# xultaeculcis/climate-super-resolution

Measured on NVIDIA B200. Metric: generator_inference_hr_mpixel_per_s, higher is better.
Workload: dtype bf16

## Files before the change

climate-super-resolution_b200/csrc/api.cu:

```cuda
#include <algorithm>
#include <atomic>
#include <cstdarg>
#include <cstdio>
#include <cstring>
#include <map>
#include <mutex>
#include <string>
#include <vector>

#include "../../include/climsr_b200.h"
#include "conv_tc.cuh"
#include "disc.cuh"
#include "elementwise.cuh"
#include "loss.cuh"
#include "metrics.cuh"
#include "rcan.cuh"
#include "rdb_tc.cuh"
#include "wgrad_tc.cuh"

namespace csr {

static thread_local char g_err[512] = "";
static std::atomic<long long> g_launches{0};
static int g_opt_pdl = 1;
static long long* g_trace = nullptr;
static unsigned long long* g_timeline = nullptr;
static int g_timeline_cap = 0;
static int g_opt_force_sw = 0;
static int g_opt_max_slots = 8;
static int g_opt_no_tma_store = 0;
static int g_opt_two_acc = 0;
static int g_opt_force_generic = 0;
static int g_opt_one_mma = 0;
static int g_opt_graphs = 1;
static int g_opt_graph_max_px = 1 << 21;
static int g_opt_issue_order = 1;
static int g_opt_wgrad_atomic = 1;
static int g_opt_eight_acc = 1;
static int g_opt_tall = 1;
static int g_opt_narrow_box = 1;
static int g_opt_regroup = 0;
static int g_opt_trace_cta = 0;
static int g_opt_reserve_sms = 0;
static int g_opt_l2_prefetch = 0;
static int g_dbg_dense = 0;
static int g_opt_dense_min = 2;
static int g_opt_tap_pack = 1;
static int g_opt_hyb = 1;
static int g_opt_merge_phases = 1;
static int g_opt_fuse_tail = 3;
[[maybe_unused]] static int g_opt_dense9 = 0;
static int g_opt_dense = 1;
static int g_opt_early = 1;
static int g_opt_pair = 0;
static int g_opt_no_single_group = 3;
static int g_dbg_wgrad[5] = {0, 0, 0, 0, 0};
static int g_opt_no_direct32 = 1;

static int fail(int code, const char* fmt, ...) {
  va_list ap;
  va_start(ap, fmt);
  vsnprintf(g_err, sizeof(g_err), fmt, ap);
  va_end(ap);
  return code;
}
#define CSR_CUDA(expr)                                                                          \
  do {                                                                                          \
    cudaError_t _e = (expr);                                                                    \
    if (_e != cudaSuccess) return fail(CSR_ERR_CUDA, "%s: %s", #expr, cudaGetErrorString(_e)); \
  } while (0)

static inline size_t align_up(size_t v, size_t a) { return (v + a - 1) / a * a; }
static inline int ceil_div(int a, int b) { return (a + b - 1) / b; }

struct DeviceInfo {
  bool ok = false;
  int sms = 0;
  int dev = -1;
};
static int device_info(DeviceInfo* out) {
  int dev = 0;
  CSR_CUDA(cudaGetDevice(&dev));
  static DeviceInfo cache[64];
  static std::mutex mu;
  if (dev >= 0 && dev < 64) {
    std::lock_guard<std::mutex> lock(mu);
    if (cache[dev].ok) { *out = cache[dev]; return CSR_OK; }
  }
  int major = 0, minor = 0, sms = 0;
  CSR_CUDA(cudaDeviceGetAttribute(&major, cudaDevAttrComputeCapabilityMajor, dev));
  CSR_CUDA(cudaDeviceGetAttribute(&minor, cudaDevAttrComputeCapabilityMinor, dev));
  CSR_CUDA(cudaDeviceGetAttribute(&sms, cudaDevAttrMultiProcessorCount, dev));
  if (major != 10) return fail(CSR_ERR_UNSUPPORTED, "device %d is sm_%d%d; this library is sm_100a only", dev, major, minor);
  out->ok = true;
  out->sms = sms;
  out->dev = dev;
  if (dev >= 0 && dev < 64) {
    std::lock_guard<std::mutex> lock(mu);
    cache[dev] = *out;
  }
  return CSR_OK;
}

typedef CUresult (*EncodeTiledFn)(CUtensorMap*, CUtensorMapDataType, cuuint32_t, void*, const cuuint64_t*, const cuuint64_t*,
                                  const cuuint32_t*, const cuuint32_t*, CUtensorMapInterleave, CUtensorMapSwizzle,
                                  CUtensorMapL2promotion, CUtensorMapFloatOOBfill);
// ... 281 lines not shown
    }
  }
  if (!p.pair && tma_out && tl.n_slots < 2 * p.n_kblocks && pp.n_store % 16 == 0 && io.out_C % 16 == 0 && (io.out_coff + pp.co_lo) % 16 == 0 &&
      !g_opt_no_direct32) {
    Tiling t2;
    if (choose_tiling(H, W, pp.kh, pp.kw, p.w_bytes, p.n_kblocks, 0, 0, &t2, p.box_c * 2) == CSR_OK && t2.n_slots >= 2 * p.n_kblocks) {
      tl = t2;
      p.store_mode = kStoreDirect32;
      p.stage_row_bytes = 0;
    }
  }
  p.act = io.act;
  if (io.act_upto > 0 && io.act == CSR_ACT_LRELU02) {
    const int upto = io.act_upto - pp.co_lo;
    if (upto <= 0) p.act = CSR_ACT_NONE;
    else if (upto < pp.n_store) { p.act = 3; p.act_upto = upto; }
  }
  p.n_stage = p.n_groups;
  const bool early_plain = res_bits == 0 && p.n_groups == 1 &&
      ((p.KW == 3 && p.PW == 1 && (p.act == 0 || p.act == 1 || p.act == 3)) || (p.KW == 2 && p.PW <= 1 && p.act == 1) ||
       (p.KW == 1 && p.PW == 0 && p.act == 2));
  const bool early_res = g_opt_early >= 2 && (res_bits == 1 || res_bits == 3) && !io.r1_pre && p.KW == 3 && p.PW == 1 && p.act == 0 && p.n_groups <= 2;
  if (g_opt_early && !p.pair && !p.tall_shift && tma_out && p.npad == 64 && pp.n_store == 64 && !g_opt_force_generic && (early_plain || early_res)) {
    Tiling te2, te1;
    const bool ok2 = choose_tiling(H, W, pp.kh, pp.kw, p.w_bytes, p.n_kblocks, p.stage_row_bytes, 2, &te2, p.box_c * 2) == CSR_OK;
    const bool ok1 = choose_tiling(H, W, pp.kh, pp.kw, p.w_bytes, p.n_kblocks, p.stage_row_bytes, 1, &te1, p.box_c * 2) == CSR_OK;
    const int want = std::min(2 * p.n_kblocks, 4);
    int stages = 0;
    if (ok2 && te2.n_slots >= want) stages = 2;
    else if (ok1 && (!ok2 || te1.n_slots > te2.n_slots)) stages = 1;
    else if (ok2) stages = 2;
    const Tiling& te = stages == 1 ? te1 : te2;
    if (stages && te.n_slots >= std::min(2, p.n_kblocks + 1) && (early_plain || te.n_slots > tl.n_slots || te.n_slots >= want)) {
      tl = te;
      p.early = 1;
      p.n_groups = 1;
      p.n_stage = stages;
      if (4 * p.KW * p.npad <= 512 && !g_opt_two_acc) p.n_acc = 4;
    }
  }
  {
    const bool hyb_early = (g_opt_hyb & 1) && p.early && ((p.KW == 3 && p.PW == 1) || (p.KW == 2 && p.PW <= 1));
#ifdef CSR_EXPERIMENTS
    const bool hyb_res = (g_opt_hyb & 2) && !p.early && p.KW == 3 && p.PW == 1 && p.act == 0 && (res_bits == 1 || res_bits == 3) && !io.r1_pre &&
                         p.n_groups == 2;
#else
    const bool hyb_res = false;
#endif
    if ((hyb_early || hyb_res) && !p.pair && !p.tall_shift && p.store_mode == kStoreStaged && p.npad == 64 && pp.n_store == 64 && p.box_c == 64 &&
        !p.stream_w && !g_opt_force_generic) {
      p.hyb = 1;
      const int acc_cols = (p.KW - 1) * p.npad;
      if (4 * acc_cols <= 512 && !g_opt_two_acc && (p.early || (g_opt_hyb & 4))) p.n_acc = 4;
    }
  }
  p.SW = tl.SW; p.TH = tl.TH; p.TW = tl.TW;
  p.sw_shift = 0;
  while ((1 << p.sw_shift) < p.SW) ++p.sw_shift;
  p.tiles_x = ceil_div(W, p.TW);
  p.tiles_y = ceil_div(H, p.TH << p.tall_shift);
  p.num_tiles = p.tiles_x * p.tiles_y * N;
  p.tiles_per_img = p.tiles_x * p.tiles_y;
  if ((long long)p.tiles_x * p.tiles_y * N >= (1 << 24) || p.tiles_per_img >= (1 << 16))
    return fail(CSR_ERR_UNSUPPORTED, "too many tiles (%d x %d x %d) for one launch", p.tiles_x, p.tiles_y, N);
  p.magic_img = ((1ull << 40) / (unsigned)p.tiles_per_img) + 1;
  p.magic_row = ((1ull << 40) / (unsigned)p.tiles_x) + 1;
  p.win_rows = tl.win_rows; p.win_bytes = tl.win_bytes; p.slot_bytes = tl.slot_bytes; p.n_slots = tl.n_slots;
  p.win_slot_bytes = (int)align_up(tl.win_bytes, 1024);
  p.stage_bytes = tl.stage_bytes;
  p.n_mma = g_opt_one_mma ? 1 : 2;
  p.issue_order = (p.n_mma == 2) && (g_opt_issue_order == 2 || (g_opt_issue_order == 1 && p.pair));
  int cols = 32;
  while (cols < p.n_acc * (p.hyb ? p.KW - 1 : p.KW) * p.npad) cols *= 2;
  if (cols > 512 || p.KW * p.npad > 256) return fail(CSR_ERR_UNSUPPORTED, "KW*npad = %d exceeds the UMMA N / TMEM budget", p.KW * p.npad);
  p.tmem_cols = cols;
  p.trace = g_trace;
  p.trace_cta = g_opt_trace_cta;
  p.use_pdl = g_opt_pdl;
  p.l2_prefetch = ((size_t)N * H * W * io.in_C * 2 > (size_t)48 << 20) ? g_opt_l2_prefetch : 0;
  p.force_generic = g_opt_force_generic;
  p.r1_pre = io.r1 ? io.r1_pre : 0;
  p.s1 = io.s1; p.s2 = io.s2;
  p.r1 = io.r1; p.r1_C = io.r1_C; p.r1_coff = io.r1_coff + pp.co_lo;
  p.r2 = io.r2; p.r2_C = io.r2_C; p.r2_coff = io.r2_coff + pp.co_lo;
  p.gate = io.gate; p.gate_C = io.gate_C; p.gate_coff = io.gate_coff + pp.co_lo; p.gate_from = io.gate_from - pp.co_lo; p.gate_neg = io.gate_neg;
  if ((io.r1 || io.r2 || io.gate) && up != 1) return fail(CSR_ERR_UNSUPPORTED, "residual / gate operands are not supported on nearest-x2 layers");
  p.out = io.out; p.out_C = io.out_C; p.out_coff = io.out_coff + pp.co_lo;
  p.out_sy = p.out_sx = up;
  p.out_oy = pp.phase >= 0 ? (pp.phase >> 1) : 0;
  p.out_ox = pp.phase >= 0 ? (pp.phase & 1) : 0;
  p.out_H = up * H; p.out_W = up * W;
  cl->w_off = pp.w_off; cl->b_off = pp.b_off;
  if (conv_smem_bytes(p) > (size_t)kSmemLimit) return fail(CSR_ERR_UNSUPPORTED, "conv needs %zu bytes of shared memory", conv_smem_bytes(p));
  return encode_act_map(&cl->tmap, io.in, N, H, W, io.in_C, p.SW, p.win_rows, p.box_c);
}

struct WgradLaunch {
  WgradParams p;
  CUtensorMap tx0, tx1, tg0, tg1;
};

static int build_wgrad(int sms, int N, int H, int W, int KW, int PW, int dy_off, int n_dy, const void* x, int x_C, int xc0, const void* gA, int gA_C,
                       int gA_c0, const void* gB, int gB_C, int gB_c0, int n_cols, float* dacc, long part_stride, int ld_n, WgradLaunch* wl) {
  if (n_cols % 16 || n_cols < 16 || n_cols > 128) return fail(CSR_ERR_UNSUPPORTED, "wgrad: n_cols %d", n_cols);
  if (x_C % 8 || gA_C % 8 || xc0 % 8 || gA_c0 % 8) return fail(CSR_ERR_BAD_ARG, "wgrad: channel pitch/offset must be multiples of 8");
  WgradParams& p = wl->p;
// ... 437 lines not shown
          ConvLaunch stub;
          memset(&stub.p, 0, sizeof(stub.p));
          stub.dense = (int)P->dense.size();
          P->dense.push_back(dl);
          P->convs.push_back(stub);
          li += 4;
          goto conv5;
        }
      }
      for (int k = 1; k <= 4; ++k) {
        ConvIO io = io_of(src, C, src, C, nf + (k - 1) * gc, CSR_ACT_LRELU02);
        if (g_opt_regroup) {
          if (k == 1) {
            io.act_upto = gc;
          } else {
            io.cin_off = nf;
            io.r1 = src; io.r1_C = C; io.r1_coff = nf + (k - 1) * gc; io.r1_pre = 1;
          }
        }
        rc = add(h, w, io);
        if (rc) return rc;
      }
    conv5:
      ConvIO io = io_of(src, C, dst, C, 0, CSR_ACT_NONE);
      io.r1 = src; io.r1_C = C; io.s1 = 0.2f;
      if (r == 2) { io.r2 = cat(3 * i); io.r2_C = C; io.s2 = 0.2f; }
      rc = add(h, w, io);
      if (rc) return rc;
    }
  }
  void* trunk_out = P->train ? cat(3 * d.nb) : cat(0);
  {
    ConvIO io = io_of(trunk_out, C, t0, 64, 0, CSR_ACT_NONE);
    io.r1 = fea0; io.r1_C = 64; io.s1 = 1.f;
    rc = add(h, w, io);
    if (rc) return rc;
  }
  rc = add(h, w, io_of(t0, 64, m1, 64, 0, CSR_ACT_LRELU02));
  if (rc) return rc;
  rc = add(2 * h, 2 * w, io_of(m1, 64, hrA, 64, 0, CSR_ACT_LRELU02));
  if (rc) return rc;
  const int H = 4 * h, W = 4 * w;
  rc = add(H, W, io_of(hrA, 64, hrB, 64, 0, CSR_ACT_LRELU02));
  if (rc) return rc;
  {
    ConvLaunch& hc = P->convs.back();
    const PackLayer& pt = packs.back();
    bool fused = false;
    if ((g_opt_fuse_tail & 2) && !P->train && hc.p.early && hc.p.KW == 3 && hc.p.PW == 1 && hc.p.npad == 64 && hc.p.stage_row_bytes == 128 &&
        pt.parts.size() == 1 && pt.parts[0].npad == 16 && pt.parts[0].w_bytes == 2048 && pt.cin_pad == 64) {
      ConvParams q = hc.p;
      q.fuse2 = 2; q.w2_bytes = pt.parts[0].w_bytes; q.n2 = 9; q.out2 = hrB; q.out2_plane = (long long)N * H * W;
      if (q.hyb) q.n_acc = 2;
      int cols = 32;
      while (cols < q.n_acc * (q.hyb ? 2 : q.KW) * q.npad + 16) cols *= 2;
      q.tmem_cols = cols;
      if (cols <= 512 && conv_smem_bytes(q) <= (size_t)kSmemLimit && (size_t)9 * N * H * W * sizeof(float) <= (size_t)N * H * W * 64 * 2) {
        hc.p = q;
        hc.w2_off = pt.parts[0].w_off;
        ConvLaunch ts;
        memset(&ts.p, 0, sizeof(ts.p));
        ts.tapsum = 1; ts.taps = reinterpret_cast<const float*>(hrB); ts.tap_plane = (long)N * H * W; ts.tap_H = H; ts.tap_W = W;
        ts.b_off = packs[li].parts[0].b_off;
        P->convs.push_back(ts);
        ++li;
        fused = true;
      }
    }
    if (!fused) {
      ConvIO io = io_of(hrB, 64, P->tlast, 1, 0, CSR_ACT_NONE);
      io.out_kind = kOutF32Planar;
      rc = add(H, W, io);
      if (rc) return rc;
    }
  }
  P->idx_srcnn1 = (int)P->convs.size();
  P->srcnn_pitch = P->train ? 64 : 32;
  const int sp = P->srcnn_pitch;
  rc = add(H, W, io_of(hrC, sp, hrD, 64, 0, CSR_ACT_RELU));
  if (rc) return rc;
  {
    ConvLaunch& c1 = P->convs.back();
    const PackLayer& p2 = packs[li];
    bool fused = false;
    if ((g_opt_fuse_tail & 1) && !P->train && c1.p.early && c1.p.KW == 1 && c1.p.PW == 0 && c1.p.npad == 64 && c1.p.stage_row_bytes == 128 &&
        p2.parts.size() == 1 && p2.parts[0].npad == 32 && p2.parts[0].w_bytes == 4096 && p2.cin_pad == 64 && sp % 8 == 0) {
      ConvParams q = c1.p;
      q.fuse2 = 1; q.w2_bytes = p2.parts[0].w_bytes; q.n2 = 32; q.out2 = hrE; q.out2_C = sp; q.out2_coff = 0;
      int cols = 32;
      while (cols < q.n_acc * q.KW * q.npad + 32) cols *= 2;
      q.tmem_cols = cols;
      if (cols <= 512 && conv_smem_bytes(q) <= (size_t)kSmemLimit) {
        c1.p = q;
        c1.w2_off = p2.parts[0].w_off; c1.b2_off = p2.parts[0].b_off;
        ++li;
        fused = true;
      }
    }
    if (!fused) {
      rc = add(H, W, io_of(hrD, 64, hrE, sp, 0, CSR_ACT_RELU));
      if (rc) return rc;
    }
  }
  {
    ConvIO io = io_of(hrE, sp, nullptr, 1, 0, CSR_ACT_NONE);
    io.out_kind = kOutF32Planar;
// ... 321 lines not shown

using namespace csr;

extern "C" {

int csr_abi_version(void) { return CSR_ABI_VERSION; }
const char* csr_last_error(void) { return g_err; }

int csr_device_check(void) {
  int n = 0;
  cudaError_t e = cudaGetDeviceCount(&n);
  if (e != cudaSuccess || n == 0) return fail(CSR_ERR_CUDA, "no CUDA device: %s", cudaGetErrorString(e));
  DeviceInfo di;
  return device_info(&di);
}

int csr_set_option(int32_t key, int32_t value) {
#ifndef CSR_EXPERIMENTS
  if ((key == 13 && value != 0) || (key == 16 && value != 0) || (key == 8 && value == 0) || (key == 32 && value != 0) || (key == 35 && (value & ~1)))
    return fail(CSR_ERR_UNSUPPORTED, "option %d=%d selects an experimental kernel variant: rebuild with CSR_EXPERIMENTS=1 python build.py --force", key, value);
#endif
  switch (key) {
    case 1: g_opt_pdl = value ? 1 : 0; return CSR_OK;
    case 2: g_opt_force_sw = value; return CSR_OK;
    case 3: g_opt_max_slots = value < 1 ? 1 : value; return CSR_OK;
    case 4: g_opt_no_tma_store = value ? 1 : 0; return CSR_OK;
    case 5: g_opt_two_acc = value ? 1 : 0; return CSR_OK;
    case 6: g_opt_force_generic = value ? 1 : 0; return CSR_OK;
    case 7: g_opt_one_mma = value ? 1 : 0; return CSR_OK;
    case 8: g_opt_no_direct32 = value ? 1 : 0; return CSR_OK;
    case 9: g_opt_no_single_group = value; return CSR_OK;
    case 11: g_opt_graphs = value ? 1 : 0; return CSR_OK;
    case 12: g_opt_graph_max_px = value; return CSR_OK;
    case 13: g_opt_pair = value; return CSR_OK;
    case 14: g_opt_issue_order = value; return CSR_OK;
    case 15: g_opt_trace_cta = value; return CSR_OK;
    case 16: g_opt_regroup = value ? 1 : 0; return CSR_OK;
    case 17: g_opt_narrow_box = value ? 1 : 0; return CSR_OK;
    case 18: g_opt_tall = value ? 1 : 0; return CSR_OK;
    case 19: g_opt_eight_acc = value ? 1 : 0; return CSR_OK;
    case 20: case 21: case 22: case 23: case 24: g_dbg_wgrad[key - 20] = value; return CSR_OK;
    case 25: g_opt_wgrad_atomic = value ? 1 : 0; return CSR_OK;
    case 27: g_opt_dense = value ? 1 : 0; return CSR_OK;
    case 36: g_opt_tap_pack = value ? 1 : 0; return CSR_OK;
    case 35: g_opt_hyb = value; return CSR_OK;
    case 34: g_opt_merge_phases = value ? 1 : 0; return CSR_OK;
    case 33: g_opt_fuse_tail = value & 3; return CSR_OK;
    case 32: g_opt_dense9 = value ? 1 : 0; return CSR_OK;
    case 31: if (value < 0 || value > 64) return fail(CSR_ERR_BAD_ARG, "option 31: windows per SM in [0, 64]"); g_opt_dense_min = value; return CSR_OK;
    case 28: g_dbg_dense = value; return CSR_OK;
    case 29: g_opt_l2_prefetch = value; return CSR_OK;
    case 30: g_opt_reserve_sms = value < 0 ? 0 : value; return CSR_OK;
    case 26: g_opt_early = value; return CSR_OK;
    default: return fail(CSR_ERR_BAD_ARG, "unknown option key %d", key);
  }
}

int64_t csr_kernel_launch_count(void) { return g_launches.load(); }

int csr_has_experiments(void) {
#ifdef CSR_EXPERIMENTS
  return 1;
#else
  return 0;
#endif
}

int csr_debug_set_trace(void* device_buffer) {
#ifdef CSR_ENABLE_TRACE
  g_trace = reinterpret_cast<long long*>(device_buffer);
  return CSR_OK;
#else
  if (!device_buffer) return CSR_OK;
  return fail(CSR_ERR_UNSUPPORTED, "this build has no pipeline tracing (rebuild with CSR_BUILD_TRACE=1 python build.py --force)");
#endif
}

int csr_debug_set_timeline(void* device_u64, int32_t capacity_launches) {
  g_timeline = reinterpret_cast<unsigned long long*>(device_u64);
  g_timeline_cap = device_u64 ? capacity_launches : 0;
  return CSR_OK;
}

int csr_num_layers(const CsrNetDesc* net) {
  int rc = check_net(net);
  if (rc) return rc;
  return (int)layer_table(*net).size();
}

int csr_layer_shape(const CsrNetDesc* net, int32_t i, int32_t shape4[4], char* name, size_t name_cap) {
  int rc = check_net(net);
  if (rc) return rc;
  const auto t = layer_table(*net);
  if (i < 0 || i >= (int)t.size() || !shape4) return fail(CSR_ERR_BAD_ARG, "layer index %d out of range", i);
  shape4[0] = t[i].cout; shape4[1] = t[i].cin; shape4[2] = t[i].kh; shape4[3] = t[i].kw;
  if (name && name_cap) snprintf(name, name_cap, "%s", t[i].name.c_str());
  return CSR_OK;
}

size_t csr_packed_weight_bytes(const CsrNetDesc* net) {
  if (check_net(net)) return 0;
  size_t total = 0;
  const auto t = layer_table(*net);
  pack_layout(fwd_exec_table(*net, t), &total);
  return total;
}
// ... 821 lines not shown
```

climate-super-resolution_b200/csrc/conv_tc.cu:

```cuda
#include <cstdio>

#include "conv_tc.cuh"
#include "ptx.cuh"

namespace csr {

namespace {

#ifdef CSR_ENABLE_TRACE
#define CSR_TRACE(role, tile_it, ev)                                                                                  \
  do {                                                                                                                \
    if (p.trace && blockIdx.x == p.trace_cta && (tile_it) < 64) p.trace[((role) * 64 + (tile_it)) * 8 + (ev)] = clock64();      \
  } while (0)
#else
#define CSR_TRACE(role, tile_it, ev) do { } while (0)
#endif

struct Tile {
  int n, y0, x0;
};

__device__ __forceinline__ int fast_div(int t, unsigned long long magic) {
  return static_cast<int>((static_cast<unsigned long long>(static_cast<unsigned>(t)) * magic) >> 40);
}
// ... 35 lines not shown
    const int src = (lane + delta) & 31;
#pragma unroll
    for (int j = 0; j < 8; ++j) s[j] = __uint_as_float(__shfl_sync(0xffffffffu, raw[j], src));
  }
#pragma unroll
  for (int j = 0; j < 8; j += 2) {
    const float2 t = __fadd2_rn(make_float2(acc[j], acc[j + 1]), make_float2(s[j], s[j + 1]));
    acc[j] = t.x;
    acc[j + 1] = t.y;
  }
}

__device__ __forceinline__ void fma_residual8(float (&v)[8], const uint4& r, float scale) {
  const uint32_t w[4] = {r.x, r.y, r.z, r.w};
#pragma unroll
  for (int i = 0; i < 4; ++i) {
    const float2 t = __ffma2_rn(make_float2(v[2 * i], v[2 * i + 1]), make_float2(scale, scale), make_float2(bf16lo(w[i]), bf16hi(w[i])));
    v[2 * i] = t.x;
    v[2 * i + 1] = t.y;
  }
}

__device__ __forceinline__ void gate8(float (&v)[8], const uint4& g, float neg) {
  const uint32_t w[4] = {g.x, g.y, g.z, g.w};
#pragma unroll
  for (int i = 0; i < 4; ++i) {
    v[2 * i] *= (bf16lo(w[i]) > 0.f) ? 1.f : neg;
    v[2 * i + 1] *= (bf16hi(w[i]) > 0.f) ? 1.f : neg;
  }
}

__device__ __forceinline__ uint4 ldg16(const void* base, size_t pix, int C, int coff) {
  return __ldg(reinterpret_cast<const uint4*>(reinterpret_cast<const __nv_bfloat16*>(base) + pix * C + coff));
}

}

template <int KW_T, int PW_T, int ACT_T, int RES_T, int ST_T, int PAIR_T = 0, int TALL_T = 0, int EARLY_T = 0, int FUSE_T = 0, int HYB_T = 0>
__global__ void __launch_bounds__(kConvThreads, 1)
conv_tc_kernel(const ConvParams p, const __grid_constant__ CUtensorMap tmap) {
  extern __shared__ uint8_t smem_raw[];
  const uint32_t smem_base = (smem_u32(smem_raw) + 1023u) & ~1023u;
  const uint32_t slots_addr = smem_base;
  const uint32_t stage_addr = slots_addr + static_cast<uint32_t>(p.n_slots) * p.slot_bytes;
  const uint32_t w_addr = stage_addr + static_cast<uint32_t>(p.n_stage) * p.stage_bytes;
  const uint32_t crank = PAIR_T ? cluster_ctarank() : 0u;
  const int w_local = p.stream_w ? 0 : (PAIR_T ? (p.w_bytes >> 1) : p.w_bytes);
  const uint32_t w2_addr = w_addr + ((w_local + 127) & ~127);
  const uint32_t b2_addr = w2_addr + (FUSE_T ? static_cast<uint32_t>(p.w2_bytes) : 0u);
  const uint32_t bias_addr = b2_addr + (FUSE_T ? 128u : 0u);
  const uint32_t bar_addr = bias_addr + 256;
  const int S = p.n_slots;
  const int NA = p.n_acc;
  const int NG = p.n_groups;
  const int wpg = kEpilogueWarps / NG;
  auto bar_w = bar_addr;
  auto bar_a_full = [&](int s) { return bar_addr + 8u * (1 + s); };
  auto bar_a_empty = [&](int s) { return bar_addr + 8u * (1 + S + s); };
  auto bar_acc_full = [&](int b) { return bar_addr + 8u * (1 + 2 * S + b); };
  auto bar_acc_empty = [&](int b) { return bar_addr + 8u * (9 + 2 * S + b); };
  auto bar_token = [&](int w) { return bar_addr + 8u * (17 + 2 * S + w); };
  const uint32_t bar_d2 = bar_addr + 8u * (19 + 2 * S);
  const uint32_t tmem_slot_addr = bar_addr + 8u * (20 + 2 * S);
  const uint32_t lead_off = PAIR_T ? (map_to_cta(bar_addr, 0) - bar_addr) : 0u;
  uint8_t* smem_gen = smem_raw + (smem_base - smem_u32(smem_raw));
  float* bias_s = reinterpret_cast<float*>(smem_gen + (bias_addr - smem_base));
  volatile uint32_t* tmem_slot = reinterpret_cast<volatile uint32_t*>(smem_gen + (tmem_slot_addr - smem_base));
  volatile uint32_t* progress = tmem_slot + 1;

  const int warp = threadIdx.x >> 5;
  const int lane = threadIdx.x & 31;
  const int KW = KW_T ? KW_T : p.KW;
  const int ph_eff = p.PH + static_cast<int>(blockIdx.y) * p.part_ph;
  const int oy_eff = p.out_oy + static_cast<int>(blockIdx.y) * p.part_oy;

  griddep_launch_dependents();

  if (threadIdx.x == 0) {
    progress[0] = 0;
    progress[1] = 0;
    mbar_init(bar_token(0), 1);
    mbar_init(bar_token(1), 1);
    mbar_init(bar_d2, 1);
    tma_prefetch_desc(&tmap);
    mbar_init(bar_w, (PAIR_T && crank == 0) ? 2 : 1);
    for (int s = 0; s < S; ++s) {
      mbar_init(bar_a_full(s), 1);
      mbar_init(bar_a_empty(s), 1);
    }
    for (int b = 0; b < NA; ++b) {
      mbar_init(bar_acc_full(b), 1);
      mbar_init(bar_acc_empty(b), PAIR_T ? 2 * wpg : wpg);
    }
    fence_mbar_init();
    fence_proxy_async_smem();
  }
  if constexpr (PAIR_T) cluster_sync_all();
  if (threadIdx.x == 0 && !p.stream_w) {
    const uint8_t* wsrc = reinterpret_cast<const uint8_t*>(p.wpk) + static_cast<size_t>(blockIdx.y) * p.part_w_bytes;
    if constexpr (PAIR_T) {
      const int full = (KW_T ? KW_T : p.KW) * p.npad * 32, half = full >> 1;
      mbar_arrive_expect_tx(bar_w, w_local);
      for (int off = 0, loc = 0; off < p.w_bytes; off += full, loc += half)
        bulk_load(w_addr + loc, wsrc + off + crank * half, half, bar_w);
    } else {
      mbar_arrive_expect_tx(bar_w, p.w_bytes + (FUSE_T ? p.w2_bytes : 0));
      for (int off = 0; off < p.w_bytes; off += 32768) {
// ... 161 lines not shown
              }
              if (last_kb && hh == 0) umma_commit(bar_acc_full(buf));
            }
          }
          if (last_kb) CSR_TRACE(1, it, 4);
          if constexpr (PAIR_T) {
            umma_commit_pair(bar_a_empty(slot));
            if (last_kb) umma_commit_pair(bar_acc_full(buf));
          } else {
            umma_commit(bar_a_empty(slot));
            if (last_kb) umma_commit(bar_acc_full(buf + tall - 1));
          }
          if (kb == p.n_kblocks - 1) CSR_TRACE(1, it, 5);
        }
        __syncwarp();
        if (kb == p.n_kblocks - 1 && lane == 0) {
          if (p.issue_order) mbar_arrive(bar_token(mw));
          CSR_TRACE(1, it, 3);
        }
        ring_advance(1);
      }
      if (p.n_mma > 1) {
        ring_advance(p.n_kblocks);
        entry += p.n_kblocks;
      }
      buf += p.n_mma * tall;
      if (buf >= NA) { buf -= NA; acc_phase ^= 1; }
      if (lane == 0) CSR_TRACE(1, it, 6);
    }
  } else {
    const int ew = warp - 1 - kMmaWarps;
    const int g = ew / wpg;
    const int wj = ew - g * wpg;
    const int lane_grp = warp & 3;
    const int sub = wj >> 2;
    const int cstep = wpg >> 2;
    const int gthreads = wpg * 32;
    const bool tracer = (ew == 0 && lane == 0);
    const int m = lane_grp * 32 + lane;
    const int ty = m >> p.sw_shift;
    const int tx = m & (p.SW - 1);
    const int n_chunks = ST_T == 3 ? 1 : p.npad >> 3;
    const int PW = KW_T ? PW_T : p.PW;
    const bool col_ok = (tx >= PW) && (tx < PW + p.TW);
    const int srow = ty * p.TW + (tx - PW);
    const int act = ACT_T >= 0 ? ACT_T : p.act;
    const bool has_r1 = RES_T >= 0 ? (RES_T & 1) != 0 : p.r1 != nullptr;
    const bool has_r2 = RES_T >= 0 ? (RES_T & 2) != 0 : p.r2 != nullptr;
    const bool has_gate = RES_T >= 0 ? (RES_T & 4) != 0 : p.gate != nullptr;
    const bool r1_pre = RES_T >= 0 ? (RES_T & 8) != 0 : p.r1_pre != 0;
    const bool tma_store = ST_T >= 0 ? ST_T == 1 : (p.store_mode == kStoreStaged);
    const bool need_pix = !tma_store || has_r1 || has_r2 || has_gate;
    const uint32_t swz = (p.stage_row_bytes == 128) ? static_cast<uint32_t>(srow & 7) : 0u;
    const uint32_t srow_addr = stage_addr + static_cast<uint32_t>(g) * p.stage_bytes + static_cast<uint32_t>(srow * p.stage_row_bytes);
    const uint32_t sbuf = stage_addr + static_cast<uint32_t>(g) * p.stage_bytes;
    const uint32_t t_lane = tmem_base + (static_cast<uint32_t>(lane_grp * 32) << 16);
    const int d0 = -PW, d1 = 1 - PW, d2 = 2 - PW;
    const int rp = p.stage_row_bytes >> 4;
    const int n_pieces = p.TH * p.TW * rp;
    uint32_t pc_s[4], pc_d[4], pc_yx[4];
    if (tma_store) {
      const int tid_g = wj * 32 + lane;
#pragma unroll
      for (int k = 0; k < 4; ++k) {
        const int i = tid_g + k * gthreads;
        const int sr = i / rp, c = i - sr * rp;
        const int dy = sr / p.TW, dx = sr - dy * p.TW;
        const uint32_t z = (p.stage_row_bytes == 128) ? static_cast<uint32_t>(sr & 7) : 0u;
        pc_s[k] = sbuf + static_cast<uint32_t>(sr * p.stage_row_bytes) + ((static_cast<uint32_t>(c) ^ z) << 4);
        pc_d[k] = static_cast<uint32_t>((dy * p.out_sy * p.out_W + dx * p.out_sx) * p.out_C + c * 8);
        pc_yx[k] = (i < n_pieces) ? ((static_cast<uint32_t>(dy) << 16) | static_cast<uint32_t>(dx)) : 0xffffffffu;
      }
    }
    int buf = g % NA;
    uint32_t acc_phase = 0;
    if constexpr (EARLY_T) {
      static_assert(KW_T >= 1 && KW_T <= 3 && (RES_T == 0 || RES_T == 1 || RES_T == 3) && ST_T == 1 && PAIR_T == 0 && TALL_T == 0,
                    "early-release epilogue: wide layers without gate / pre-activation addend");
      const int ch_lo = sub * 16;
      uint32_t sb = 0;
      const bool two_stage = p.n_stage == 2;
      constexpr int N2 = FUSE_T == 1 ? 32 : 16;
      Tile prev_tl = {0, 0, 0};
      int n_done = 0;
      auto consume_d2 = [&](const Tile& t2) {
        tc_fence_after();
        if constexpr (FUSE_T == 1) {
          uint32_t r2[8];
          tmem_ld8(t_lane + static_cast<uint32_t>(NA * nacc) + sub * 8, r2);
          tmem_ld_wait();
          tc_fence_before();
          const int y = t2.y0 + ty, x = t2.x0 - PW_T + tx;
          if (col_ok && y < p.H && x < p.W && sub * 8 < p.n2) {
            const float* bias2_s = reinterpret_cast<const float*>(smem_gen + (b2_addr - smem_base)) + sub * 8;
            float v[8];
#pragma unroll
            for (int j = 0; j < 8; ++j) v[j] = fmaxf(__uint_as_float(r2[j]) + bias2_s[j], 0.f);
            __nv_bfloat16* o2 = reinterpret_cast<__nv_bfloat16*>(p.out2) + ((static_cast<size_t>(t2.n) * p.H + y) * p.W + x) * p.out2_C + p.out2_coff + sub * 8;
            *reinterpret_cast<uint4*>(o2) = make_uint4(pack_bf16x2(v[0], v[1]), pack_bf16x2(v[2], v[3]), pack_bf16x2(v[4], v[5]), pack_bf16x2(v[6], v[7]));
          }
        } else if constexpr (FUSE_T == 2) {
          if (sub < 2) {
            uint32_t r2[8];
            tmem_ld8(t_lane + static_cast<uint32_t>(NA * nacc) + sub * 8, r2);
            tmem_ld_wait();
            const int py = m / p.TW, px = m - py * p.TW;
            const int y = t2.y0 + py, x = t2.x0 + px;
            if (m < p.TH * p.TW && y < p.H && x < p.W) {
              float* o2 = reinterpret_cast<float*>(p.out2) + (static_cast<size_t>(t2.n) * p.H + y) * p.W + x + static_cast<size_t>(sub * 8) * p.out2_plane;
              if (sub == 0) {
#pragma unroll
                for (int j = 0; j < 8; ++j) o2[static_cast<size_t>(j) * p.out2_plane] = __uint_as_float(r2[j]);
              } else {
                o2[0] = __uint_as_float(r2[0]);
              }
            }
          }
          tc_fence_before();
        }
      };
      for (int it = 0; ; ++it) {
        const int t = blockIdx.x + it * static_cast<int>(gridDim.x);
        if (t >= p.num_tiles) break;
        if (tracer) CSR_TRACE(2, it, 3);
        const Tile tl = decode_tile<0>(p, t);
        uint4 q1[2], q2[2];
        if constexpr (RES_T != 0) {
          const int y = tl.y0 + ty, x = tl.x0 - PW_T + tx;
          const bool valid = col_ok && (y < p.H) && (x < p.W);
          const size_t pix = (static_cast<size_t>(tl.n) * p.H + y) * p.W + x;
#pragma unroll
          for (int jj = 0; jj < 2; ++jj) {
            const int ch0 = ch_lo + jj * 8;
            q1[jj] = valid ? ldg16(p.r1, pix, p.r1_C, p.r1_coff + ch0) : make_uint4(0, 0, 0, 0);
            if constexpr (RES_T == 3) q2[jj] = valid ? ldg16(p.r2, pix, p.r2_C, p.r2_coff + ch0) : make_uint4(0, 0, 0, 0);
          }
        }
        if (!two_stage && it > 0) named_bar_sync(1, gthreads);
        const uint32_t t_addr = t_lane + buf * nacc + ch_lo;
        mbar_wait(bar_acc_full(buf), acc_phase);
        tc_fence_after();
        if (tracer) CSR_TRACE(2, it, 1);
        constexpr int KW_E = HYB_T ? KW_T - 1 : KW_T;
        uint32_t raw[2][KW_E][8];
#pragma unroll
        for (int jj = 0; jj < 2; ++jj)
#pragma unroll
          for (int dx = 0; dx < KW_E; ++dx) tmem_ld8(t_addr + dx * p.npad + jj * 8, raw[jj][dx]);
        tmem_ld_wait();
        tc_fence_before();
        __syncwarp();
        if (lane == 0) mbar_arrive(bar_acc_empty(buf));
        if (tracer) CSR_TRACE(2, it, 0);
#pragma unroll
        for (int jj = 0; jj < 2; ++jj) {
          const int ch0 = ch_lo + jj * 8;
          float v[8];
          {
            const float4 b0 = *reinterpret_cast<const float4*>(bias_s + ch0);
            const float4 b1 = *reinterpret_cast<const float4*>(bias_s + ch0 + 4);
            v[0] = b0.x; v[1] = b0.y; v[2] = b0.z; v[3] = b0.w; v[4] = b1.x; v[5] = b1.y; v[6] = b1.z; v[7] = b1.w;
          }
#pragma unroll
          for (int dx = 0; dx < KW_E; ++dx) gather_add8(v, raw[jj][dx], dx - PW_T, lane);
          if (act == 3) {
            if (ch0 < p.act_upto) apply_act8(v, 1);
          } else {
            apply_act8(v, act);
          }
          if constexpr (RES_T != 0) fma_residual8(v, q1[jj], p.s1);
          if constexpr (RES_T == 3) fma_residual8(v, q2[jj], p.s2);
          if (col_ok && ch0 < p.n_store)
            st_shared_v4(srow_addr + sb * p.stage_bytes + ((static_cast<uint32_t>(ch0 >> 3) ^ swz) << 4), pack_bf16x2(v[0], v[1]),
                         pack_bf16x2(v[2], v[3]), pack_bf16x2(v[4], v[5]), pack_bf16x2(v[6], v[7]));
        }
        if (tracer) CSR_TRACE(2, it, 4);
        if constexpr (FUSE_T) {
          if (two_stage && it > 0) {
            mbar_wait_spin(bar_d2, static_cast<uint32_t>(it - 1) & 1u);
            consume_d2(prev_tl);
          }
          fence_proxy_async_smem();
        }
        named_bar_sync(1, gthreads);
        if (tracer) CSR_TRACE(2, it, 7);
        if constexpr (FUSE_T) {
          if (warp == 1 + kMmaWarps) {
            if (it == 0) mbar_wait_spin(bar_w, 0);
            tc_fence_after();
            if (elect_one()) {
              const uint32_t a16 = ((stage_addr + sb * p.stage_bytes) >> 4) | ((16u >> 4) << 16);
              const uint32_t a_hi2 = (1024u >> 4) | (1u << 14) | (2u << 29);
              const uint32_t b16 = (w2_addr >> 4) | ((128u >> 4) << 16);
              const uint32_t b_hi2 = (256u >> 4) | (1u << 14);
              const uint32_t idesc2 = make_idesc_bf16(kTileM, N2);
#pragma unroll
              for (int ks = 0; ks < 4; ++ks)
                umma_bf16_split(tmem_base + static_cast<uint32_t>(NA * nacc), a16 + ks * 2, a_hi2, b16 + ks * ((N2 * 32) >> 4), b_hi2, idesc2, ks ? 1u : 0u);
              umma_commit(bar_d2);
            }
            __syncwarp();
          }
          if (!two_stage) {
            mbar_wait_spin(bar_d2, static_cast<uint32_t>(it) & 1u);
            consume_d2(tl);
          }
          prev_tl = tl;
          n_done = it + 1;
        } else {
        __nv_bfloat16* tile_out = reinterpret_cast<__nv_bfloat16*>(p.out) +
            ((static_cast<size_t>(tl.n) * p.out_H + (tl.y0 * p.out_sy + oy_eff)) * p.out_W + (tl.x0 * p.out_sx + p.out_ox)) * p.out_C +
            p.out_coff + static_cast<int>(blockIdx.y) * p.part_c;
        const uint32_t lim = (static_cast<uint32_t>(max(0, min(p.H - tl.y0, 0x7fff))) << 16) | static_cast<uint32_t>(min(p.W - tl.x0, 0x7fff));
#pragma unroll
        for (int k = 0; k < 2; ++k) {
          const bool ok = ((pc_yx[k] >> 16) < (lim >> 16)) && ((pc_yx[k] & 0xffffu) < (lim & 0xffffu));
          if (ok) {
            const uint4 val = ld_shared_v4(pc_s[k] + sb * p.stage_bytes);
            *reinterpret_cast<uint4*>(tile_out + pc_d[k]) = val;
            if constexpr (KW_T == 3 && ACT_T == 0 && RES_T == 0 && FUSE_T == 0) {
              if (p.out_dup) {
                const uint32_t pixoff = ((pc_yx[k] >> 16) * p.out_sy * p.out_W + (pc_yx[k] & 0xffffu) * p.out_sx);
                __nv_bfloat16* dup = reinterpret_cast<__nv_bfloat16*>(p.out_dup) +
                    ((static_cast<size_t>(tl.n) * p.out_H + (tl.y0 * p.out_sy + oy_eff)) * p.out_W + (tl.x0 * p.out_sx + p.out_ox)) * p.dup_C + p.dup_coff;
                *reinterpret_cast<uint4*>(dup + static_cast<size_t>(pixoff) * p.dup_C + (pc_d[k] - pixoff * p.out_C)) = val;
              }
            }
          }
        }
        }
        if (tracer) CSR_TRACE(2, it, 2);
        if (two_stage) sb ^= 1u;
        if (++buf >= NA) { buf = 0; acc_phase ^= 1; }
      }
      if constexpr (FUSE_T) {
        if (two_stage && n_done > 0) {
          mbar_wait_spin(bar_d2, static_cast<uint32_t>(n_done - 1) & 1u);
          consume_d2(prev_tl);
        }
      }
    } else
    for (int it = g; ; it += NG) {
      const int t = blockIdx.x + (it >> TALL_T) * static_cast<int>(gridDim.x);
      if (t >= p.num_tiles) break;
      if (tracer) CSR_TRACE(2, it, 3);
      Tile tl = decode_tile<TALL_T>(p, t);
      if constexpr (TALL_T) tl.y0 += (it & 1) * p.TH;
      bool valid = false;
      size_t pix = 0;
      int y = 0, x = 0;
      uint4 q1[4], q2[4];
      if (need_pix) {
        y = tl.y0 + ty;
        x = tl.x0 - PW + tx;
        valid = col_ok && (y < p.H) && (x < p.W);
        pix = (static_cast<size_t>(tl.n) * p.H + y) * p.W + x;
#pragma unroll
        for (int j = 0; j < 4; ++j) {
          const int ch0 = (2 * (sub + (j >> 1) * cstep) + (j & 1)) * 8;
          const bool on = valid && (ch0 < p.n_store);
          q1[j] = (on && has_r1) ? ldg16(p.r1, pix, p.r1_C, p.r1_coff + ch0) : make_uint4(0, 0, 0, 0);
          if (has_gate)
            q2[j] = (on && ch0 >= p.gate_from) ? ldg16(p.gate, pix, p.gate_C, p.gate_coff + ch0)
                                               : make_uint4(0x3f803f80u, 0x3f803f80u, 0x3f803f80u, 0x3f803f80u);
          else
            q2[j] = (on && has_r2) ? ldg16(p.r2, pix, p.r2_C, p.r2_coff + ch0) : make_uint4(0, 0, 0, 0);
        }
      }
      if (tma_store) named_bar_sync(1 + g, gthreads);
      if (tracer) CSR_TRACE(2, it, 0);
      const uint32_t t_addr = t_lane + buf * nacc;
      mbar_wait(bar_acc_full(buf), acc_phase);
      tc_fence_after();
      if (tracer) CSR_TRACE(2, it, 1);
      uint4 held = make_uint4(0, 0, 0, 0);
#pragma unroll
      for (int j = 0; j < 4; ++j) {
        const int c = 2 * (sub + (j >> 1) * cstep) + (j & 1);
        if (c < n_chunks) {
          const int ch0 = c * 8;
          float v[8];
          {
            const float4 b0 = *reinterpret_cast<const float4*>(bias_s + ch0);
            const float4 b1 = *reinterpret_cast<const float4*>(bias_s + ch0 + 4);
            v[0] = b0.x; v[1] = b0.y; v[2] = b0.z; v[3] = b0.w; v[4] = b1.x; v[5] = b1.y; v[6] = b1.z; v[7] = b1.w;
          }
// ... 154 lines not shown
  attr[1].val.clusterDim.x = 2;
  attr[1].val.clusterDim.y = 1;
  attr[1].val.clusterDim.z = 1;
  cfg.attrs = attr;
  cfg.numAttrs = PAIR_T ? 2 : 1;
  return static_cast<int>(cudaLaunchKernelEx(&cfg, kern, p, tmap));
}

int launch_conv_tc(const ConvParams& p, const CUtensorMap& tmap, int num_sms, cudaStream_t stream) {
  const int res = (p.r1 ? 1 : 0) | (p.r2 ? 2 : 0) | (p.gate ? 4 : 0) | ((p.r1 && p.r1_pre) ? 8 : 0);
  if ((res & 6) == 6) return static_cast<int>(cudaErrorInvalidValue);
  if (p.pair) {
#ifdef CSR_EXPERIMENTS
    if (p.store_mode != kStoreStaged || p.KW != 3 || p.PW != 1 || p.act != 0 || (p.num_tiles & 1) || p.force_generic)
      return static_cast<int>(cudaErrorInvalidValue);
    switch (res) {
      case 1: return launch_t<3, 1, 0, 1, 1, 1>(p, tmap, num_sms, stream);
      case 3: return launch_t<3, 1, 0, 3, 1, 1>(p, tmap, num_sms, stream);
      case 4: return launch_t<3, 1, 0, 4, 1, 1>(p, tmap, num_sms, stream);
      case 5: return launch_t<3, 1, 0, 5, 1, 1>(p, tmap, num_sms, stream);
      default: return static_cast<int>(cudaErrorInvalidValue);
    }
#else
    return static_cast<int>(cudaErrorNotSupported);
#endif
  }
  if (p.tall_shift) {
    if ((p.n_acc != 4 && p.n_acc != 8) || p.n_groups != 4) return static_cast<int>(cudaErrorInvalidValue);
    if (p.store_mode == kStoreStaged && !p.force_generic && p.KW == 3 && p.PW == 1 && p.act == 1 && res == 0)
      return launch_t<3, 1, 1, 0, 1, 0, 1>(p, tmap, num_sms, stream);
#ifdef CSR_EXPERIMENTS
    if (p.store_mode == kStoreStaged && !p.force_generic && p.KW == 3 && p.PW == 1 && p.act == 1 && res == 9)
      return launch_t<3, 1, 1, 9, 1, 0, 1>(p, tmap, num_sms, stream);
#endif
    if (p.store_mode == kStoreStaged && !p.force_generic && p.KW == 1 && p.PW == 0 && p.act == 2 && res == 0)
      return launch_t<1, 0, 2, 0, 1, 0, 1>(p, tmap, num_sms, stream);
    if (p.store_mode == kStoreStaged && !p.force_generic && p.KW == 3 && p.PW == 1 && p.act == 0 && res == 4)
      return launch_t<3, 1, 0, 4, 1, 0, 1>(p, tmap, num_sms, stream);
    if (p.store_mode == kStoreStaged && !p.force_generic && p.KW == 3 && p.PW == 1 && p.act == 0 && res == 5)
      return launch_t<3, 1, 0, 5, 1, 0, 1>(p, tmap, num_sms, stream);
    if (p.store_mode == kStoreStaged && !p.force_generic && p.KW == 1 && p.PW == 0 && p.act == 0 && res == 4)
      return launch_t<1, 0, 0, 4, 1, 0, 1>(p, tmap, num_sms, stream);
    if (p.store_mode == kStoreF32Planar && !p.force_generic && p.KW == 3 && p.PW == 1 && p.act == 0 && res == 0)
      return launch_t<3, 1, 0, 0, 3, 0, 1>(p, tmap, num_sms, stream);
    if (p.store_mode == kStoreF32Planar && !p.force_generic && p.KW == 5 && p.PW == 2 && p.act == 0 && res == 0)
      return launch_t<5, 2, 0, 0, 3, 0, 1>(p, tmap, num_sms, stream);
    switch (p.KW) {
      case 1: return launch_t<1, 0, -1, -1, -1, 0, 1>(p, tmap, num_sms, stream);
      case 3: if (p.PW == 1) return launch_t<3, 1, -1, -1, -1, 0, 1>(p, tmap, num_sms, stream);
      default: return launch_t<0, 0, -1, -1, -1, 0, 1>(p, tmap, num_sms, stream);
    }
  }
  if (p.early) {
    if (p.store_mode != kStoreStaged || p.n_groups != 1 || p.n_stage < 1 || p.n_stage > 2 || p.npad != 64 || p.force_generic)
      return static_cast<int>(cudaErrorInvalidValue);
    if (p.fuse2 == 2) {
      if (p.KW != 3 || p.PW != 1 || p.act != 1 || res != 0 || p.stage_row_bytes != 128 || p.w2_bytes != 2048 || p.n2 != 9 || p.out2_plane <= 0 ||
          p.tmem_cols < p.n_acc * (p.hyb ? p.KW - 1 : p.KW) * p.npad + 16 || p.parts > 1)
        return static_cast<int>(cudaErrorInvalidValue);
      if (p.hyb) return launch_t<3, 1, 1, 0, 1, 0, 0, 1, 2, 1>(p, tmap, num_sms, stream);
      return launch_t<3, 1, 1, 0, 1, 0, 0, 1, 2>(p, tmap, num_sms, stream);
    }
    if (p.fuse2) {
      if (p.KW != 1 || p.PW != 0 || p.act != 2 || res != 0 || p.stage_row_bytes != 128 || p.w2_bytes != 4096 || p.n2 < 8 || p.n2 > 32 || (p.n2 & 7) ||
          p.tmem_cols < p.n_acc * p.KW * p.npad + 32 || p.parts > 1)
        return static_cast<int>(cudaErrorInvalidValue);
      return launch_t<1, 0, 2, 0, 1, 0, 0, 1, 1>(p, tmap, num_sms, stream);
    }
#define CSR_EARLY(KW_, PW_, ACT_, RES_) \
    if (p.KW == KW_ && p.PW == PW_ && p.act == ACT_ && res == RES_) {                                                                   \
      if constexpr (KW_ >= 2) { if (p.hyb) return launch_t<KW_, PW_, ACT_, RES_, 1, 0, 0, 1, 0, 1>(p, tmap, num_sms, stream); }            \
      return launch_t<KW_, PW_, ACT_, RES_, 1, 0, 0, 1>(p, tmap, num_sms, stream);                                                      \
    }
    CSR_EARLY(3, 1, 1, 0)
    CSR_EARLY(3, 1, 0, 0)
#ifdef CSR_EXPERIMENTS
    CSR_EARLY(3, 1, 3, 0)
#endif
    CSR_EARLY(2, 0, 1, 0)
    CSR_EARLY(2, 1, 1, 0)
    CSR_EARLY(1, 0, 2, 0)
    CSR_EARLY(3, 1, 0, 1)
    CSR_EARLY(3, 1, 0, 3)
#undef CSR_EARLY
    return static_cast<int>(cudaErrorInvalidValue);
  }
#define CSR_CASE(KW_, PW_, ACT_, RES_, ST_)                                                                  \
  if (p.store_mode == (ST_ == 1 ? kStoreStaged : ST_ == 3 ? kStoreF32Planar : kStoreDirect32) && !p.force_generic && p.KW == KW_ && \
      p.PW == PW_ && p.act == ACT_ && res == RES_)                                                           \
    return launch_t<KW_, PW_, ACT_, RES_, ST_>(p, tmap, num_sms, stream);
  CSR_CASE(3, 1, 1, 0, 1)
  CSR_CASE(3, 1, 0, 0, 1)
  CSR_CASE(3, 1, 4, 0, 1)
  if (p.hyb && p.store_mode == kStoreStaged && !p.force_generic && p.KW == 3 && p.PW == 1 && p.act == 0) {
#ifdef CSR_EXPERIMENTS
    if (res == 1) return launch_t<3, 1, 0, 1, 1, 0, 0, 0, 0, 1>(p, tmap, num_sms, stream);
    if (res == 3) return launch_t<3, 1, 0, 3, 1, 0, 0, 0, 0, 1>(p, tmap, num_sms, stream);
#endif
    return static_cast<int>(cudaErrorInvalidValue);
  }
  CSR_CASE(3, 1, 0, 1, 1)
  CSR_CASE(3, 1, 0, 3, 1)
#ifdef CSR_EXPERIMENTS
  CSR_CASE(3, 1, 0, 1, 2)
  CSR_CASE(3, 1, 0, 3, 2)
  CSR_CASE(3, 1, 3, 0, 1)
  CSR_CASE(3, 1, 1, 9, 1)
// ... 23 lines not shown
```

Baseline: 938.9.

## Split early-release hybrid conv epilogue into multiple independent groups

Early-release hybrid-fold convolution layers (no residual, not fused) can now run the epilogue warps as 2 or 4 independent groups. Each group handles interleaved tiles with its own staging buffers, named barrier and accumulator slots, so several tiles drain from TMEM at once. Within a group, warps walk the channels in slices and release the accumulator only after the last slice. Tiling is re-chosen for the larger staging need, and the fused tail layer is forced back to a single group, which trades shared memory and slot count for epilogue concurrency.

```diff
diff --git a/climate-super-resolution_b200/csrc/api.cu b/climate-super-resolution_b200/csrc/api.cu
--- a/climate-super-resolution_b200/csrc/api.cu
+++ b/climate-super-resolution_b200/csrc/api.cu
@@ -52,6 +52,7 @@
 [[maybe_unused]] static int g_opt_dense9 = 0;
 static int g_opt_dense = 1;
 static int g_opt_early = 1;
+static int g_opt_early_groups = 4;
 static int g_opt_pair = 0;
 static int g_opt_no_single_group = 3;
 static int g_dbg_wgrad[5] = {0, 0, 0, 0, 0};
@@ -439,6 +440,19 @@
       p.hyb = 1;
       const int acc_cols = (p.KW - 1) * p.npad;
       if (4 * acc_cols <= 512 && !g_opt_two_acc && (p.early || (g_opt_hyb & 4))) p.n_acc = 4;
+    }
+  }
+  const int early_groups = (g_opt_early_groups == 4 && p.KW != 2) ? 2 : g_opt_early_groups;
+  if (p.early && p.hyb && res_bits == 0 && early_groups > 1 && p.n_acc % early_groups == 0) {
+    for (int per_group = 2; per_group >= 1; --per_group) {
+      Tiling tg;
+      if (choose_tiling(H, W, pp.kh, pp.kw, p.w_bytes, p.n_kblocks, p.stage_row_bytes, early_groups * per_group, &tg, p.box_c * 2) == CSR_OK &&
+          tg.n_slots >= std::min(2 * p.n_kblocks, 4)) {
+        tl = tg;
+        p.n_groups = early_groups;
+        p.n_stage = early_groups * per_group;
+        break;
+      }
     }
   }
   p.SW = tl.SW; p.TH = tl.TH; p.TW = tl.TW;
@@ -982,6 +996,13 @@
       ConvParams q = hc.p;
       q.fuse2 = 2; q.w2_bytes = pt.parts[0].w_bytes; q.n2 = 9; q.out2 = hrB; q.out2_plane = (long long)N * H * W;
       if (q.hyb) q.n_acc = 2;
+      if (q.n_groups > 1) {
+        Tiling t1;
+        q.n_groups = 1;
+        q.n_stage = 2;
+        if (choose_tiling(H, W, q.KH, q.KW, q.w_bytes, q.n_kblocks, q.stage_row_bytes, q.n_stage, &t1, q.box_c * 2) == CSR_OK && t1.SW == q.SW)
+          q.n_slots = t1.n_slots;
+      }
       int cols = 32;
       while (cols < q.n_acc * (q.hyb ? 2 : q.KW) * q.npad + 16) cols *= 2;
       q.tmem_cols = cols;
@@ -1409,6 +1430,10 @@
     case 29: g_opt_l2_prefetch = value; return CSR_OK;
     case 30: g_opt_reserve_sms = value < 0 ? 0 : value; return CSR_OK;
     case 26: g_opt_early = value; return CSR_OK;
+    case 37:
+      if (value != 1 && value != 2 && value != 4) return fail(CSR_ERR_BAD_ARG, "option 37: epilogue groups of the early-release hybrid-fold layers, 1, 2 or 4");
+      g_opt_early_groups = value;
+      return CSR_OK;
     default: return fail(CSR_ERR_BAD_ARG, "unknown option key %d", key);
   }
 }
diff --git a/climate-super-resolution_b200/csrc/conv_tc.cu b/climate-super-resolution_b200/csrc/conv_tc.cu
--- a/climate-super-resolution_b200/csrc/conv_tc.cu
+++ b/climate-super-resolution_b200/csrc/conv_tc.cu
@@ -111,7 +111,8 @@
   const uint32_t bar_addr = bias_addr + 256;
   const int S = p.n_slots;
   const int NA = p.n_acc;
-  const int NG = p.n_groups;
+  constexpr bool kEarlyOneGroup = EARLY_T && !(HYB_T && RES_T == 0 && FUSE_T == 0);
+  const int NG = kEarlyOneGroup ? 1 : p.n_groups;
   const int wpg = kEpilogueWarps / NG;
   auto bar_w = bar_addr;
   auto bar_a_full = [&](int s) { return bar_addr + 8u * (1 + s); };
@@ -379,17 +380,18 @@
     const bool tma_store = ST_T >= 0 ? ST_T == 1 : (p.store_mode == kStoreStaged);
     const bool need_pix = !tma_store || has_r1 || has_r2 || has_gate;
     const uint32_t swz = (p.stage_row_bytes == 128) ? static_cast<uint32_t>(srow & 7) : 0u;
-    const uint32_t srow_addr = stage_addr + static_cast<uint32_t>(g) * p.stage_bytes + static_cast<uint32_t>(srow * p.stage_row_bytes);
-    const uint32_t sbuf = stage_addr + static_cast<uint32_t>(g) * p.stage_bytes;
+    const uint32_t sbuf = stage_addr + static_cast<uint32_t>(p.n_stage > NG ? 2 * g : g) * p.stage_bytes;
+    const uint32_t srow_addr = sbuf + static_cast<uint32_t>(srow * p.stage_row_bytes);
     const uint32_t t_lane = tmem_base + (static_cast<uint32_t>(lane_grp * 32) << 16);
     const int d0 = -PW, d1 = 1 - PW, d2 = 2 - PW;
     const int rp = p.stage_row_bytes >> 4;
     const int n_pieces = p.TH * p.TW * rp;
-    uint32_t pc_s[4], pc_d[4], pc_yx[4];
+    constexpr int kMaxPieces = (EARLY_T && !kEarlyOneGroup && KW_T == 2) ? 8 : 4;
+    uint32_t pc_s[kMaxPieces], pc_d[kMaxPieces], pc_yx[kMaxPieces];
     if (tma_store) {
       const int tid_g = wj * 32 + lane;
 #pragma unroll
-      for (int k = 0; k < 4; ++k) {
+      for (int k = 0; k < kMaxPieces; ++k) {
         const int i = tid_g + k * gthreads;
         const int sr = i / rp, c = i - sr * rp;
         const int dy = sr / p.TW, dx = sr - dy * p.TW;
@@ -404,9 +406,11 @@
     if constexpr (EARLY_T) {
       static_assert(KW_T >= 1 && KW_T <= 3 && (RES_T == 0 || RES_T == 1 || RES_T == 3) && ST_T == 1 && PAIR_T == 0 && TALL_T == 0,
                     "early-release epilogue: wide layers without gate / pre-activation addend");
+      const int qw = wpg >> 2;
+      const int n_slice = kEarlyOneGroup ? 1 : 4 / qw;
       const int ch_lo = sub * 16;
       uint32_t sb = 0;
-      const bool two_stage = p.n_stage == 2;
+      const bool two_stage = p.n_stage == 2 * NG;
       constexpr int N2 = FUSE_T == 1 ? 32 : 16;
       Tile prev_tl = {0, 0, 0};
       int n_done = 0;
@@ -446,7 +450,8 @@
           tc_fence_before();
         }
       };
-      for (int it = 0; ; ++it) {
+      for (int seq = 0; ; ++seq) {
+        const int it = g + seq * NG;
         const int t = blockIdx.x + it * static_cast<int>(gridDim.x);
         if (t >= p.num_tiles) break;
         if (tracer) CSR_TRACE(2, it, 3);
@@ -463,11 +468,14 @@
             if constexpr (RES_T == 3) q2[jj] = valid ? ldg16(p.r2, pix, p.r2_C, p.r2_coff + ch0) : make_uint4(0, 0, 0, 0);
           }
         }
-        if (!two_stage && it > 0) named_bar_sync(1, gthreads);
-        const uint32_t t_addr = t_lane + buf * nacc + ch_lo;
+        if (!two_stage && seq > 0) named_bar_sync(1 + g, gthreads);
         mbar_wait(bar_acc_full(buf), acc_phase);
         tc_fence_after();
         if (tracer) CSR_TRACE(2, it, 1);
+#pragma unroll 1
+        for (int sl = 0; sl < n_slice; ++sl) {
+        const int ch_sl = ch_lo + sl * qw * 16;
+        const uint32_t t_addr = t_lane + buf * nacc + ch_sl;
         constexpr int KW_E = HYB_T ? KW_T - 1 : KW_T;
         uint32_t raw[2][KW_E][8];
 #pragma unroll
@@ -475,13 +483,15 @@
 #pragma unroll
           for (int dx = 0; dx < KW_E; ++dx) tmem_ld8(t_addr + dx * p.npad + jj * 8, raw[jj][dx]);
         tmem_ld_wait();
-        tc_fence_before();
-        __syncwarp();
-        if (lane == 0) mbar_arrive(bar_acc_empty(buf));
-        if (tracer) CSR_TRACE(2, it, 0);
+        if (sl == n_slice - 1) {
+          tc_fence_before();
+          __syncwarp();
+          if (lane == 0) mbar_arrive(bar_acc_empty(buf));
+          if (tracer) CSR_TRACE(2, it, 0);
+        }
 #pragma unroll
         for (int jj = 0; jj < 2; ++jj) {
-          const int ch0 = ch_lo + jj * 8;
+          const int ch0 = ch_sl + jj * 8;
           float v[8];
           {
             const float4 b0 = *reinterpret_cast<const float4*>(bias_s + ch0);
@@ -501,22 +511,23 @@
             st_shared_v4(srow_addr + sb * p.stage_bytes + ((static_cast<uint32_t>(ch0 >> 3) ^ swz) << 4), pack_bf16x2(v[0], v[1]),
                          pack_bf16x2(v[2], v[3]), pack_bf16x2(v[4], v[5]), pack_bf16x2(v[6], v[7]));
         }
+        }
         if (tracer) CSR_TRACE(2, it, 4);
         if constexpr (FUSE_T) {
-          if (two_stage && it > 0) {
-            mbar_wait_spin(bar_d2, static_cast<uint32_t>(it - 1) & 1u);
+          if (two_stage && seq > 0) {
+            mbar_wait_spin(bar_d2, static_cast<uint32_t>(seq - 1) & 1u);
             consume_d2(prev_tl);
           }
           fence_proxy_async_smem();
         }
-        named_bar_sync(1, gthreads);
+        named_bar_sync(1 + g, gthreads);
         if (tracer) CSR_TRACE(2, it, 7);
         if constexpr (FUSE_T) {
           if (warp == 1 + kMmaWarps) {
-            if (it == 0) mbar_wait_spin(bar_w, 0);
+            if (seq == 0) mbar_wait_spin(bar_w, 0);
             tc_fence_after();
             if (elect_one()) {
-              const uint32_t a16 = ((stage_addr + sb * p.stage_bytes) >> 4) | ((16u >> 4) << 16);
+              const uint32_t a16 = ((sbuf + sb * p.stage_bytes) >> 4) | ((16u >> 4) << 16);
               const uint32_t a_hi2 = (1024u >> 4) | (1u << 14) | (2u << 29);
               const uint32_t b16 = (w2_addr >> 4) | ((128u >> 4) << 16);
               const uint32_t b_hi2 = (256u >> 4) | (1u << 14);
@@ -529,18 +540,19 @@
             __syncwarp();
           }
           if (!two_stage) {
-            mbar_wait_spin(bar_d2, static_cast<uint32_t>(it) & 1u);
+            mbar_wait_spin(bar_d2, static_cast<uint32_t>(seq) & 1u);
             consume_d2(tl);
           }
           prev_tl = tl;
-          n_done = it + 1;
+          n_done = seq + 1;
         } else {
         __nv_bfloat16* tile_out = reinterpret_cast<__nv_bfloat16*>(p.out) +
             ((static_cast<size_t>(tl.n) * p.out_H + (tl.y0 * p.out_sy + oy_eff)) * p.out_W + (tl.x0 * p.out_sx + p.out_ox)) * p.out_C +
             p.out_coff + static_cast<int>(blockIdx.y) * p.part_c;
         const uint32_t lim = (static_cast<uint32_t>(max(0, min(p.H - tl.y0, 0x7fff))) << 16) | static_cast<uint32_t>(min(p.W - tl.x0, 0x7fff));
 #pragma unroll
-        for (int k = 0; k < 2; ++k) {
+        for (int k = 0; k < kMaxPieces; ++k) {
+          if (k >= 2 * n_slice) break;
           const bool ok = ((pc_yx[k] >> 16) < (lim >> 16)) && ((pc_yx[k] & 0xffffu) < (lim & 0xffffu));
           if (ok) {
             const uint4 val = ld_shared_v4(pc_s[k] + sb * p.stage_bytes);
@@ -558,7 +570,8 @@
         }
         if (tracer) CSR_TRACE(2, it, 2);
         if (two_stage) sb ^= 1u;
-        if (++buf >= NA) { buf = 0; acc_phase ^= 1; }
+        buf += NG;
+        if (buf >= NA) { buf -= NA; acc_phase ^= 1; }
       }
       if constexpr (FUSE_T) {
         if (two_stage && n_done > 0) {
@@ -819,7 +832,9 @@
     }
   }
   if (p.early) {
-    if (p.store_mode != kStoreStaged || p.n_groups != 1 || p.n_stage < 1 || p.n_stage > 2 || p.npad != 64 || p.force_generic)
+    if (p.store_mode != kStoreStaged || p.n_stage < p.n_groups || p.n_stage > 2 * p.n_groups || p.npad != 64 || p.force_generic)
+      return static_cast<int>(cudaErrorInvalidValue);
+    if (p.n_groups != 1 && ((p.n_groups != 2 && (p.n_groups != 4 || p.KW != 2)) || p.n_acc % p.n_groups || !p.hyb || res != 0 || p.fuse2 || (p.n_stage % p.n_groups)))
       return static_cast<int>(cudaErrorInvalidValue);
     if (p.fuse2 == 2) {
       if (p.KW != 3 || p.PW != 1 || p.act != 1 || res != 0 || p.stage_row_bytes != 128 || p.w2_bytes != 2048 || p.n2 != 9 || p.out2_plane <= 0 ||
```

New measurement: 945.8, median of 6. No clear change (+0.7%).
